# mathematiguy/pypardis

Hardware: AMD Instinct MI355X
Metric: points clustered/sec (whole node), 100M 3-D pts, 1/2/4/8 GPUs; % HBM roofline (higher is better)
Workload: dtype f32 coords, f64 predicate

## Files before the change

pypardis_amd/csrc/engine.hip:

```cpp
#include <cstring>
#include <rocprim/rocprim.hpp>
#ifndef PD_SORT_ROCPRIM
#define PD_SORT_ROCPRIM 0
#endif

#include <algorithm>
#include <type_traits>
#include <cmath>
#include <cstring>
#include <vector>

#include "compact.hpp"
#include "internal.hpp"
#include "pred.hpp"
#include "rsort.hpp"
#include "scan.hpp"
#include "stream.hpp"
#include "uf.hpp"

namespace pd {
namespace {

#ifndef PD_CHECK_BOUNDS
#define PD_CHECK_BOUNDS 0
// ... 1130 lines not shown
            R.lim_lo = -(int32_t)(c < 64 ? c : 64);
            const int64_t up = g.nc[0] - 1 - c;
            R.lim_hi = (int32_t)(up < 64 ? up : 64);
        } else {
            const float csf = (float)g.cs[j];
            const float shrink = 1.0f - 1.0f / 65536.0f, abs_s = csf * (1.0f / 1048576.0f);
            float dl = fmaxf(f * csf * shrink - abs_s, 0.0f);
            float dh = fmaxf((1.0f - f) * csf * shrink - abs_s, 0.0f);
            if constexpr (M == 0) {
                dl *= dl;
                dh *= dh;
            }
            R.tl[j] = c > 0 ? dl : INFINITY;
            R.th[j] = c < g.nc[j] - 1 ? dh : INFINITY;
        }
    }
    R.kc = g.base + lin;
    return R;
}

template <typename T, int D, int M, bool U>
__device__ __forceinline__ void row_range3(const Cells& C, const Count3Grid<T, D, M, U>& g,
                                           const RowGeo<D>& R, float e2, int q, uint32_t& s,
                                           uint32_t& e) {
    float d2 = 0.0f;
    int64_t koff = 0;
#pragma unroll
    for (int j = 1; j < D; ++j) {
        const int o = row_off<D>(q, j);
        d2 += o < 0 ? R.tl[j] : (o > 0 ? R.th[j] : 0.0f);
        koff += o < 0 ? -(int64_t)g.S[j] : (o > 0 ? (int64_t)g.S[j] : 0);
    }
    const bool ok = d2 <= e2;
    float w;
    if constexpr (M == 0)
        w = fmaxf(__builtin_amdgcn_sqrtf(fmaxf(e2 - d2, 0.0f)), 1.0842022e-19f);
    else
        w = fmaxf(e2 - d2, 0.0f);
    const float wc = w * g.wsc + g.wsl;
    int32_t dx0 = (int32_t)floorf(R.f0 - wc), dx1 = (int32_t)floorf(R.f0 + wc);
    dx0 = dx0 > R.lim_lo ? dx0 : R.lim_lo;
    dx1 = dx1 < R.lim_hi ? dx1 : R.lim_hi;
    const uint64_t rb = R.kc + (uint64_t)koff;
    const uint64_t k0 = ok ? rb + (uint64_t)(int64_t)dx0 : R.kc;
    const uint64_t k1 = ok ? rb + (uint64_t)(int64_t)(dx1 + 1) : R.kc;
    const uint4 w0 = dir_word(C, k0), w1 = dir_word(C, k1);
    const uint32_t i0 = dir_rank(w0, k0), i1 = dir_rank(w1, k1);
    s = C.cstart[i0];
    e = C.cstart[i1];
    e = e > s ? e : s;
}

#ifndef PD_COUNT_WPE
#define PD_COUNT_WPE 8
#endif
#ifndef PD_BORDER_WPE
#define PD_BORDER_WPE 8
#endif
constexpr int kCountWpe = PD_COUNT_WPE, kBorderWpe = PD_BORDER_WPE;
template <typename T, int D, int M, bool ST, int WPE = 1, bool REPLAY = false, bool WT = false>
__global__ __launch_bounds__(kBlock) __attribute__((amdgpu_waves_per_eu(WPE))) void count4_kernel(
    const T* __restrict__ Xs, uint32_t R, Cells C, double eps, double eps2, float lo, float hi,
    uint32_t ms, int full, uint32_t rot_min, uint8_t* __restrict__ core,
    uint32_t* __restrict__ mn_out, uint32_t* __restrict__ cnt_out,
    unsigned long long* __restrict__ stats, uint32_t rmod,
    const uint64_t* __restrict__ wrec = nullptr, uint64_t wthr = 0) {
    constexpr int NR = NRows<D>::v;
    constexpr int B = NR < 3 ? NR : 3, NB = NR / B;
    uint32_t r = rec_index();
    if (r >= R) return;
    if constexpr (REPLAY) r = r % rmod;
    (void)rmod;
    double a[D];
    load_rec<T, D>(Xs, r, a);
    const Pred<T, D, M> pr = make_pred<T, D, M>(Xs, r, a, eps, eps2, lo, hi);
    const uint32_t stop = full ? 0xFFFFFFFFu : ms;
    float e2 = M == 0 ? (float)eps2 : (float)eps;
    e2 = e2 * (1.0f + 1.0f / 65536.0f);
    uint32_t cnt = 0, mn = kNone, mn2 = kNone, n_cand = 0;
    uint64_t wsum = 0;
    const uint64_t wstop = full ? ~0ull : wthr;
    (void)wsum;
    (void)wstop;
    with_part(C.part_start, C.P, r, [&](int L, auto U) {
        Count3Grid<T, D, M, decltype(U)::value> g;
        g.load(C.parts + L);
        const RowGeo<D> geo = row_geo<T, D, M, decltype(U)::value>(g, a);
        for (int bt = 0; bt < NB; ++bt) {
            uint32_t s0, e0, s1 = 0, e1 = 0, s2 = 0, e2r = 0;
            row_range3<T, D, M, decltype(U)::value>(C, g, geo, e2, bt * B, s0, e0);
            if constexpr (B > 1) row_range3<T, D, M, decltype(U)::value>(C, g, geo, e2, bt * B + 1, s1, e1);
            if constexpr (B > 2) row_range3<T, D, M, decltype(U)::value>(C, g, geo, e2, bt * B + 2, s2, e2r);
            const uint32_t l0 = e0 - s0, l01 = l0 + (e1 - s1), tot = l01 + (e2r - s2);
            auto jpos = [&](uint32_t w) -> uint32_t {
                uint32_t j = s0 + w;
                if constexpr (B > 1) j = w >= l0 ? s1 + (w - l0) : j;
                if constexpr (B > 2) j = w >= l01 ? s2 + (w - l01) : j;
                return j;
            };
            uint32_t v0 = 0;
            if (bt == 0 && tot > rot_min) {
                const uint32_t vr = (r & ~(kRotAlign - 1u)) - s0;
                v0 = vr < l0 ? vr : 0u;
            }
            auto sweep = [&](auto ROT) -> bool {
                for (uint32_t v = 0; v < tot; v += 4) {
                    uint32_t j[4];
                    T b[4][D];
                    uint64_t wb[4];
                    (void)wb;
#pragma unroll
                    for (int u = 0; u < 4; ++u) {
                        uint32_t w = v + u;
                        if constexpr (decltype(ROT)::value) {
                            w += v0;
                            w = w >= tot ? w - tot : w;
                        }
                        j[u] = jpos(w);
                        load_raw<T, D>(Xs, v + u < tot ? j[u] : r, b[u]);
                        if constexpr (WT) wb[u] = wrec[v + u < tot ? j[u] : r];
                    }
#pragma unroll
                    for (int u = 0; u < 4; ++u) {
                        const bool h = (v + u < tot) && pr(b[u]);
                        cnt += h ? 1u : 0u;
                        if constexpr (WT) wsum += h ? wb[u] : 0ull;
                        const uint32_t x = h ? j[u] : kNone;
                        mn2 = min(mn2, max(mn, x));
                        mn = min(mn, x);
                    }
                    if constexpr (ST) n_cand += (tot - v < 4u ? tot - v : 4u);
                    if constexpr (WT) {
                        if (wsum >= wstop) return true;
                    } else {
                        if (cnt >= stop) return true;
                    }
                }
                return false;
            };
            const bool stopped = __any(v0 != 0) ? sweep(std::true_type{}) : sweep(std::false_type{});
            if (stopped) return;
        }
    });
    const bool is_core = WT ? wsum >= wthr : cnt >= ms;
    core[r] = (is_core ? 1 : 0) | (cnt >= 2 ? 2 : 0) | (cnt == 2 ? 4 : 0);
    reinterpret_cast<uint2*>(mn_out)[r] = make_uint2(mn, mn2);
    if constexpr (!WT)
        if (cnt_out) cnt_out[r] = full ? cnt : (cnt < ms ? cnt : ms);
    if constexpr (ST) atomicAdd(stats + 0, (unsigned long long)n_cand);
}

constexpr uint32_t kMixed = 0xFFFFFFFEu;

__device__ __forceinline__ uint32_t root_l1(const uint32_t* par, uint32_t x) {
    uint32_t p = ld_l1(par + x);
    while (p != x) {
        x = p;
        p = ld_l1(par + x);
    }
    return x;
}

__device__ __forceinline__ uint32_t lds_find(const uint32_t* lp, uint32_t x) {
    uint32_t p = lp[x];
    while (p != x) {
        x = p;
        p = lp[x];
    }
    return x;
}

__device__ __forceinline__ void lds_union(uint32_t* lp, uint32_t a, uint32_t b) {
    while (true) {
        a = lds_find(lp, a);
        b = lds_find(lp, b);
        if (a == b) return;
        if (a > b) {
            const uint32_t t = a;
            a = b;
            b = t;
        }
        if (atomicCAS(lp + b, b, a) == b) return;
    }
}

template <typename T, int D, int M, int W, bool ST>
__global__ __launch_bounds__(kBlock) void window_uf_kernel(const T* __restrict__ Xs, uint32_t R,
                                                           double eps, double eps2, float lo,
                                                           float hi, uint32_t* __restrict__ par,
                                                           unsigned long long* __restrict__ stats) {
    constexpr int E = 64 + W;
    static_assert(E <= 128, "two slots per lane");
    __shared__ T sx[kBlock / 64][E][D];
    __shared__ uint32_t sp[kBlock / 64][E];
    __shared__ uint32_t lp[kBlock / 64][E];
    const int lane = threadIdx.x & 63, w = threadIdx.x >> 6;
    const uint32_t b = xcd_block(blockIdx.x, gridDim.x) * kBlock + w * 64;
    for (int e = lane; e < E; e += 64) {
        const uint32_t j = b + e;
        T v[D];
        uint32_t p = kNone;
        if (j < R) {
            load_raw<T, D>(Xs, j, v);
            p = ld_l1(par + j);
            if (p != kNone && p != j) {
                const uint32_t root = root_l1(par, p);
                if (e < 64 && root != p) st_rlx(par + j, root);
                p = root;
            }
        } else {
#pragma unroll
            for (int k = 0; k < D; ++k) v[k] = T(0);
        }
#pragma unroll
        for (int k = 0; k < D; ++k) sx[w][e][k] = v[k];
        sp[w][e] = p;
        lp[w][e] = (uint32_t)e;
    }
    __syncthreads();
    const uint32_t r = b + lane;
    const uint32_t p0 = r < R ? sp[w][lane] : kNone;
    LinkStats st;
    if (p0 != kNone) {
        Pred<T, D, M> pr;
#pragma unroll
        for (int k = 0; k < D; ++k) {
            pr.ar[k] = sx[w][lane][k];
            pr.a[k] = (double)pr.ar[k];
        }
        pr.eps = eps;
        pr.eps2 = eps2;
        pr.lo = lo;
        pr.hi = hi;
#pragma unroll 4
        for (int k = 1; k <= W; ++k) {
            const uint32_t pj = sp[w][lane + k];
            if (pj == kNone || pj == p0 || r + k >= R) continue;
            T bj[D];
#pragma unroll
            for (int q = 0; q < D; ++q) bj[q] = sx[w][lane + k][q];
            if constexpr (ST) ++st.cand;
            if (pr(bj)) {
                if constexpr (ST) ++st.hit;
                lds_union(lp[w], (uint32_t)lane, (uint32_t)(lane + k));
            }
        }
    }
    __syncthreads();
    for (int e = lane; e < E; e += 64) {
        const uint32_t pe = sp[w][e];
        if (pe == kNone) continue;
        const uint32_t lr = lds_find(lp[w], (uint32_t)e);
        const uint32_t pl = sp[w][lr];
        if (pl == pe) continue;
        if (e > 0 && sp[w][e - 1] == pe && lds_find(lp[w], (uint32_t)(e - 1)) == lr) continue;
        if constexpr (ST) ++st.unions;
        uf_link_roots(par, uf_find_l1(par, pl), uf_find_l1(par, pe));
    }
    if constexpr (ST) {
        const uint32_t c = block_sum_u32(st.cand), h = block_sum_u32(st.hit),
                       u = block_sum_u32(st.unions);
        if (threadIdx.x == 0) {
            atomicAdd(stats + 1, (unsigned long long)c);
            atomicAdd(stats + 2, (unsigned long long)h);
            atomicAdd(stats + 6, (unsigned long long)u);
        }
    }
}

__device__ __forceinline__ uint32_t root_merge(uint32_t a, uint32_t b) {
    return a == kNone ? b : (b == kNone ? a : (a == b ? a : kMixed));
}

__device__ __forceinline__ uint32_t core_root(uint32_t* __restrict__ par, uint32_t r) {
    const uint32_t p0 = par[r];
    if (p0 == kNone) return kNone;
    uint32_t p = p0;
    while (true) {
        const uint32_t q = par[p];
        if (q == p) break;
        p = q;
    }
    if (p != p0) par[r] = p;
    return p;
}

__device__ __forceinline__ void word_merge(uint32_t* wroot, uint64_t w, uint32_t v) {
    if (v == kNone) return;
    uint32_t cur = ld_rlx(wroot + w);
    while (true) {
        const uint32_t want = root_merge(cur, v);
        if (want == cur) return;
        const uint32_t prev = atomicCAS(wroot + w, cur, want);
        if (prev == cur) return;
        cur = prev;
    }
}

constexpr uint32_t kMidCell = 16, kWordBig = 1024;

template <typename K, bool W32>
__global__ __launch_bounds__(kBlock) void cell_word_root_kernel(
    const uint32_t* __restrict__ cstart, const uint32_t* __restrict__ ncells,
    const K* __restrict__ ckeys, uint32_t* __restrict__ par, uint32_t* __restrict__ croot,
    uint32_t* __restrict__ wroot, uint32_t* __restrict__ mid, uint32_t* __restrict__ nmid,
    uint32_t* __restrict__ big, uint32_t* __restrict__ nbig, const uint4* __restrict__ pages) {
    const uint32_t c = blockIdx.x * kBlock + threadIdx.x;
    const int lane = threadIdx.x & 63;
    const uint32_t nc = *ncells;
    if (c - (uint32_t)lane >= nc) return;
    using WT = std::conditional_t<W32, uint32_t, uint64_t>;
    uint32_t v = kNone;
    WT word = (WT)~0ull;
    uint32_t sz = 0, s = 0;
    if (c < nc) {
        s = cstart[c];
        sz = cstart[c + 1] - s;
        word = (WT)word_slot(pages, (uint64_t)ckeys[c]);
    }
    wave_append(mid, nmid, sz > kMidCell && sz <= kWordBig, c);
    wave_append(big, nbig, sz > kWordBig, c);
    if (c < nc && sz <= kMidCell) {
        for (uint32_t b = s; b < s + sz; b += 4) {
            uint32_t p0[4], p1[4];
#pragma unroll
            for (int q = 0; q < 4; ++q) p0[q] = b + q < s + sz ? par[b + q] : kNone;
#pragma unroll
            for (int q = 0; q < 4; ++q) p1[q] = p0[q] != kNone ? par[p0[q]] : kNone;
#pragma unroll
            for (int q = 0; q < 4; ++q) {
                if (p0[q] == kNone) continue;
                uint32_t x = p0[q];
                if (p1[q] != x) {
                    x = p1[q];
                    while (true) {
                        const uint32_t y = par[x];
                        if (y == x) break;
                        x = y;
                    }
                    par[b + q] = x;
                }
                v = root_merge(v, x);
            }
        }
        croot[c] = v;
    }
#pragma unroll
    for (int o = 1; o < 64; o <<= 1) {
        const uint32_t nv = (uint32_t)__shfl_up((int)v, o, 64);
        const WT nw = shfl_up_w(word, o);
        if (lane >= o && nw == word) v = root_merge(v, nv);
    }
    const WT next = shfl_down_w(word, 1);
    if (c < nc && (lane == 63 || next != word)) word_merge(wroot, (uint64_t)word, v);
}

template <typename K>
__global__ __launch_bounds__(kBlock) void mid_cell_word_root_kernel(
    const uint32_t* __restrict__ cstart, const K* __restrict__ ckeys,
    const uint32_t* __restrict__ mid, const uint32_t* __restrict__ nmid,
    uint32_t* __restrict__ par, uint32_t* __restrict__ croot, uint32_t* __restrict__ wroot,
    const uint4* __restrict__ pages) {
    const uint32_t lane = threadIdx.x & 63;
    const uint32_t nm = *nmid;
    const uint32_t nw = gridDim.x * (kBlock / 64);
    for (uint32_t i = (blockIdx.x * kBlock + threadIdx.x) >> 6; i < nm; i += nw) {
        const uint32_t c = mid[i];
        const uint32_t s = cstart[c], e = cstart[c + 1];
        uint32_t v = kNone;
        for (uint32_t r = s + lane; r < e; r += 64) v = root_merge(v, core_root(par, r));
#pragma unroll
        for (int o = 32; o > 0; o >>= 1) v = root_merge(v, (uint32_t)__shfl_xor((int)v, o, 64));
        if (lane == 0) {
            croot[c] = v;
            word_merge(wroot, word_slot(pages, (uint64_t)ckeys[c]), v);
        }
    }
}

template <typename K>
__global__ __launch_bounds__(kBlock) void big_cell_word_root_kernel(
    const uint32_t* __restrict__ cstart, const K* __restrict__ ckeys,
    const uint32_t* __restrict__ big, const uint32_t* __restrict__ nbig,
    uint32_t* __restrict__ par, uint32_t* __restrict__ croot, uint32_t* __restrict__ wroot,
    const uint4* __restrict__ pages) {
    __shared__ uint32_t part[kBlock / 64];
    const uint32_t nb = *nbig;
    for (uint32_t i = blockIdx.x; i < nb; i += gridDim.x) {
        const uint32_t c = big[i];
        const uint32_t e = cstart[c + 1];
        uint32_t v = kNone;
        for (uint32_t r = cstart[c] + threadIdx.x; r < e; r += kBlock) v = root_merge(v, core_root(par, r));
#pragma unroll
        for (int o = 32; o > 0; o >>= 1) v = root_merge(v, (uint32_t)__shfl_xor((int)v, o, 64));
        if ((threadIdx.x & 63) == 0) part[threadIdx.x >> 6] = v;
        __syncthreads();
        if (threadIdx.x == 0) {
            uint32_t w = kNone;
#pragma unroll
            for (int k = 0; k < kBlock / 64; ++k) w = root_merge(w, part[k]);
            croot[c] = w;
            word_merge(wroot, word_slot(pages, (uint64_t)ckeys[c]), w);
        }
        __syncthreads();
// ... 793 lines not shown
    } else {
        PD_HIP(hipMemsetAsync(cstart, 0, sizeof(uint32_t), s));
        PD_HIP(hipMemsetAsync(dncells, 0, sizeof(uint32_t), s));
    }
    uint64_t cgrid0 = R;
#if PD_NC_SYNC
    if (R) {
        uint32_t* hnc = (uint32_t*)((char*)pinned(ctx, 16) + 8);
        PD_HIP(hipMemcpyAsync(hnc, dncells, sizeof(uint32_t), hipMemcpyDeviceToHost, s));
        uint32_t* hwb = hnc + 1;
        if (wbad) PD_HIP(hipMemcpyAsync(hwb, wbad, sizeof(uint32_t), hipMemcpyDeviceToHost, s));
        sync(s);
        cgrid0 = std::max<uint64_t>(1, std::min<uint64_t>(*hnc, R));
        if (wbad && *hwb)
            throw Error(-1, "sample_weight: " + std::to_string(*hwb) +
                                " value(s) not finite or outside [0, 2^31]");
        wbad = nullptr;
    }
#endif
    if (wbad) {
        uint32_t* hwb = (uint32_t*)pinned(ctx, sizeof(uint32_t));
        PD_HIP(hipMemcpyAsync(hwb, wbad, sizeof(uint32_t), hipMemcpyDeviceToHost, s));
        sync(s);
        if (*hwb)
            throw Error(-1, "sample_weight: " + std::to_string(*hwb) +
                                " value(s) not finite or outside [0, 2^31]");
    }
    auto prefix_words = [&](uint4* d, uint64_t nw, bool read_total) -> uint64_t {
        const unsigned wtiles = (unsigned)std::max<uint64_t>(1, (nw + 4 * kBlock - 1) / (4 * kBlock));
        uint32_t* wcnt = ctx.arena.get<uint32_t>("tile_cnt", (size_t)wtiles + 1);
        uint64_t* woff = ctx.arena.get<uint64_t>("tile_off", (size_t)wtiles + 1);
        hipLaunchKernelGGL(dir_tile_kernel, dim3(wtiles), dim3(kBlock), 0, s, d, nw, wcnt);
        const uint64_t tot = tile_offsets(ctx, wcnt, wtiles, woff, s, read_total);
        hipLaunchKernelGGL(dir_write_kernel, dim3(wtiles), dim3(kBlock), 0, s, d, nw, woff);
        return tot;
    };
    uint64_t W;
    uint4* dir;
    uint4* pages = nullptr;
    if (!a.dir_paged) {
        W = (Gtot >> 6) + 2;
        dir = ctx.arena.get<uint4>("dir", W);
        PD_HIP(hipMemsetAsync(dir, 0, sizeof(uint4) * W, s));
        if (R) {
            if (sizeof(K) == 4 || key_bits <= 37)
                hipLaunchKernelGGL((dir_bits_kernel<K, 0, true>), dim3(blocks(cgrid0)), dim3(kBlock), 0, s,
                                   ckeys, dncells, dir);
            else
                hipLaunchKernelGGL((dir_bits_kernel<K, 0, false>), dim3(blocks(cgrid0)), dim3(kBlock), 0,
                                   s, ckeys, dncells, dir);
        }
        prefix_words(dir, W, false);
    } else {
        const uint64_t NP = (Gtot >> 12) + 2;
        pages = ctx.arena.get<uint4>("dir_pages", NP);
        PD_HIP(hipMemsetAsync(pages, 0, sizeof(uint4) * NP, s));
        if (R) {
            if (sizeof(K) == 4 || key_bits <= 43)
                hipLaunchKernelGGL((dir_bits_kernel<K, 6, true>), dim3(blocks(cgrid0)), dim3(kBlock), 0, s,
                                   ckeys, dncells, pages);
            else
                hipLaunchKernelGGL((dir_bits_kernel<K, 6, false>), dim3(blocks(cgrid0)), dim3(kBlock), 0,
                                   s, ckeys, dncells, pages);
        }
        if (R && !PD_NC_SYNC)
            PD_HIP(hipMemcpyAsync((char*)pinned(ctx, 16) + 8, dncells, sizeof(uint32_t),
                                  hipMemcpyDeviceToHost, s));
        const uint64_t nw = prefix_words(pages, NP, true);
        W = nw + 1;
        dir = ctx.arena.get<uint4>("dir", W);
        if (R)
        {
            const uint32_t nch = *(const uint32_t*)((const char*)pinned(ctx, 16) + 8);
            const uint64_t wg = std::max<uint64_t>(1, std::min<uint64_t>(nch, R));
            if (sizeof(K) == 4 || key_bits <= 37)
                hipLaunchKernelGGL((word_write_kernel<K, true>), dim3(blocks(wg)), dim3(kBlock), 0, s,
                                   ckeys, dncells, pages, dir);
            else
                hipLaunchKernelGGL((word_write_kernel<K, false>), dim3(blocks(wg)), dim3(kBlock), 0, s,
                                   ckeys, dncells, pages, dir);
        }
        else
            PD_HIP(hipMemsetAsync(dir, 0, sizeof(uint4), s));
    }
    ctx.t.dir_words = (int64_t)W;
    PD_HIP(hipGetLastError());
    tm.mark();

    Cells C{parts, part_start, P, dir, cstart, pages};
    const double eps = a.eps, eps2 = a.eps * a.eps;
    float slo = -1.0f, shi = INFINITY;
    {
        const double thr = a.metric == 0 ? eps2 : eps;
        if (std::is_same<T, float>::value && thr > 1e-30 && thr < 1e30 && ctx.screen) {
            slo = std::nextafter((float)(thr * (1.0 - 1.0 / 262144.0)), 0.0f);
            shi = std::nextafter((float)(thr * (1.0 + 1.0 / 262144.0)), INFINITY);
        }
    }
    uint8_t* core = ctx.arena.get<uint8_t>("core", R);
    uint32_t* mn = ctx.arena.get<uint32_t>("minnbr", 2 * (size_t)R);
    uint32_t* cnt_rec = a.counts ? ctx.arena.get<uint32_t>("cnt_rec", R) : nullptr;
    unsigned long long* sst = nullptr;
    if (ctx.sweep_stats) {
        sst = ctx.arena.get<unsigned long long>("sweep_stats", 10);
        PD_HIP(hipMemsetAsync(sst, 0, sizeof(unsigned long long) * 10, s));
    }
    uint32_t* h_nc = nullptr;
    hipEvent_t ev_nc = nullptr;
    if (R && ctx.centre_window < 0) {
        h_nc = (uint32_t*)pinned(ctx, sizeof(uint32_t));
        PD_HIP(hipEventCreateWithFlags(&ev_nc, hipEventDisableTiming));
        PD_HIP(hipMemcpyAsync(h_nc, dncells, sizeof(uint32_t), hipMemcpyDeviceToHost, s));
        PD_HIP(hipEventRecord(ev_nc, s));
    }
    if (R) {
        const uint32_t rot = ctx.count_rotate ? (uint32_t)ctx.count_rotate : 0xFFFFFFFFu;
        if (wrec)
            launch_count_weighted<T, D, M>(s, Xs, R, C, eps, eps2, slo, shi, (uint32_t)a.min_samples,
                                           ctx.full_counts ? 1 : 0, rot, core, mn, wrec);
        else if (sst)
            launch_count<T, D, M, true>(s, Xs, R, C, eps, eps2, slo, shi, (uint32_t)a.min_samples,
                                        ctx.full_counts ? 1 : 0, rot, core, mn, cnt_rec, sst);
        else
            launch_count<T, D, M, false>(s, Xs, R, C, eps, eps2, slo, shi, (uint32_t)a.min_samples,
                                         ctx.full_counts ? 1 : 0, rot, core, mn, cnt_rec, sst);
        if (ctx.count_replay > 0 && !sst && !wrec)
            ctx.t.count_kernel = replay_count<T, D, M>(
                s, Xs, R, (uint32_t)ctx.count_replay, C, eps, eps2, slo, shi,
                (uint32_t)a.min_samples, ctx.full_counts ? 1 : 0, rot, core, mn, cnt_rec);
    }
    PD_HIP(hipGetLastError());
    tm.mark();

    uint32_t* par = ctx.arena.get<uint32_t>("parent", R);
    uint32_t* gmin = ctx.arena.get<uint32_t>("gmin", R);
    if (R) {
        uint32_t* wroot = ctx.arena.get<uint32_t>("word_root", W);
        const uint64_t NW = a.phase == 0 ? (n + 31) / 32 : 0;
        const uint64_t NWz = NW ? ((NW + 31) & ~uint64_t(31)) + kRootLists * kRootCntStride : 0;
        uint32_t* kbits = NW ? ctx.arena.get<uint32_t>("key_bits", NWz) : nullptr;
        hipLaunchKernelGGL(init_kernel, dim3(sub_blocks(std::max<uint64_t>(std::max<uint64_t>(R, W), NWz))),
                           dim3(kBlock), 0, s, R, core, mn, 1, par, gmin, wroot, (uint64_t)W, kbits, NWz);
        int cw = ctx.centre_window;
        uint64_t cgrid = R;
        if (cw < 0) {
            PD_HIP(hipEventSynchronize(ev_nc));
            (void)hipEventDestroy(ev_nc);
            const uint32_t nc = *h_nc ? *h_nc : 1u;
            cgrid = std::min<uint64_t>(nc, R);
            cw = 2 * (uint64_t)R <= 5ull * nc ? 2 : ((uint64_t)R <= 8ull * nc ? 8 : 16);
        }
        auto go = [&](auto Wc) {
            constexpr int Wv = decltype(Wc)::value;
            if (sst)
                hipLaunchKernelGGL((window_uf_kernel<T, D, M, Wv, true>), dim3(blocks(R)),
                                   dim3(kBlock), 0, s, Xs, R, eps, eps2, slo, shi, par, sst);
            else
                hipLaunchKernelGGL((window_uf_kernel<T, D, M, Wv, false>), dim3(blocks(R)),
                                   dim3(kBlock), 0, s, Xs, R, eps, eps2, slo, shi, par, sst);
        };
        if (cw <= 2)
            go(std::integral_constant<int, 2>{});
        else if (cw <= 4)
            go(std::integral_constant<int, 4>{});
        else if (cw <= 8)
            go(std::integral_constant<int, 8>{});
        else if (cw <= 16)
            go(std::integral_constant<int, 16>{});
        else if (cw <= 32)
            go(std::integral_constant<int, 32>{});
        else
            go(std::integral_constant<int, 64>{});
        uint32_t* croot = ctx.arena.get<uint32_t>("cell_root", R);
        {
            uint32_t* big = ctx.arena.get<uint32_t>("big_cells", R / (kWordBig + 1) + 1);
            uint32_t* mid = ctx.arena.get<uint32_t>("mid_cells", R / (kMidCell + 1) + 1);
            uint32_t* nbig = ctrs + 8;
            if ((uint64_t)W < 0xFFFFFFFFull)
                hipLaunchKernelGGL((cell_word_root_kernel<K, true>), dim3(blocks(cgrid)), dim3(kBlock), 0,
                                   s, cstart, dncells, ckeys, par, croot, wroot, mid, nbig + 1, big,
                                   nbig, pages);
            else
                hipLaunchKernelGGL((cell_word_root_kernel<K, false>), dim3(blocks(cgrid)), dim3(kBlock),
                                   0, s, cstart, dncells, ckeys, par, croot, wroot, mid, nbig + 1,
                                   big, nbig, pages);
            hipLaunchKernelGGL((mid_cell_word_root_kernel<K>), dim3(2048), dim3(kBlock), 0, s,
                               cstart, ckeys, mid, nbig + 1, par, croot, wroot, pages);
            hipLaunchKernelGGL((big_cell_word_root_kernel<K>), dim3(1024), dim3(kBlock), 0, s,
                               cstart, ckeys, big, nbig, par, croot, wroot, pages);
        }
        const uint32_t pcap = (uint32_t)std::min<uint64_t>(R, 64ull << 20);
        uint2* plist = ctx.arena.get<uint2>("pair_list", pcap);
        uint32_t* pcount = ctrs + 10;
        const unsigned vtiles = blocks(cgrid);
        uint8_t* vflag = ctx.arena.get<uint8_t>("verify_flags", R);
        uint32_t* vlist = ctx.arena.get<uint32_t>("verify_list", R);
        uint32_t* vcnt = ctx.arena.get<uint32_t>("tile_cnt", (size_t)vtiles + 1);
        uint64_t* voff = ctx.arena.get<uint64_t>("tile_off", (size_t)vtiles + 1);
        if (ctx.verify_fused) {
            hipLaunchKernelGGL((cell_verify_kernel<T, D, M, K>), dim3(vtiles), dim3(kBlock), 0, s,
                               Xs, keys, nullptr, 0u, croot, wroot, C, xsub_of(ctx), eps, eps2,
                               slo, shi, par, plist, pcap, pcount, sst, dncells);
        } else {
            hipLaunchKernelGGL((verify_screen_kernel<D, K>), dim3(vtiles), dim3(kBlock), 0, s, keys,
                               dncells, croot, wroot, C, xsub_of(ctx), vflag, vcnt);
            const uint32_t NV = (uint32_t)tile_offsets(ctx, vcnt, vtiles, voff, s, true);
            if (NV) {
                hipLaunchKernelGGL(flag_list_kernel, dim3(vtiles), dim3(kBlock), 0, s, vflag, dncells,
                                   voff, vlist);
                hipLaunchKernelGGL((cell_verify_kernel<T, D, M, K>), dim3(blocks(NV)), dim3(kBlock), 0,
                                   s, Xs, keys, vlist, NV, croot, wroot, C, xsub_of(ctx), eps, eps2,
                                   slo, shi, par, plist, pcap, pcount, sst, nullptr);
            }
        }
        hipLaunchKernelGGL((pair_kernel<T, D, M>), dim3(std::min(blocks(pcap), 4096u)), dim3(kBlock), 0, s, Xs, plist,
                           pcount, pcap, cstart, croot, eps, eps2, slo, shi, par);
    }
    PD_HIP(hipGetLastError());
    tm.mark();
    if (P > 1 && R) {
        const unsigned gb = std::min(blocks(R), 2048u);
        hipLaunchKernelGGL(rep_kernel, dim3(gb), dim3(kBlock), 0, s, dup_list, lcount, vals, par,
                           rep);
        hipLaunchKernelGGL(merge_kernel, dim3(gb), dim3(kBlock), 0, s, dup_list, lcount, vals, rep,
                           par);
    }
    tm.mark();
    if (R) {
        const unsigned rb = sub_blocks(R, kRootSub);
        const uint32_t seg = ((rb + kRootLists - 1) / kRootLists) * (uint32_t)(kRootSub * kBlock);
        const uint64_t NW = a.phase == 0 ? (n + 31) / 32 : 0;
        uint32_t* rlist = NW ? ctx.arena.get<uint32_t>("root_list", (size_t)seg * kRootLists) : nullptr;
        uint32_t* rcnt = NW ? ctx.arena.get<uint32_t>("key_bits", 1) + ((NW + 31) & ~uint64_t(31))
                            : nullptr;
        hipLaunchKernelGGL(roots_kernel, dim3(rb), dim3(kBlock), 0, s, R, vals, a.gid, par, gmin, rlist,
                           rcnt, seg, lcount + 1, ctx.sweep_stats ? 1 : 0);
        if (a.phase == 0) {
            uint32_t* kbits = ctx.arena.get<uint32_t>("key_bits", 1);
            uint32_t* kpre = ctx.arena.get<uint32_t>("key_pre", NW);
            const unsigned gb = kRootLists * 16;
            hipLaunchKernelGGL(root_mark_kernel, dim3(gb), dim3(kBlock), 0, s, rlist, rcnt, seg, gmin,
                               kbits);
            rocprim::transform_iterator<const uint32_t*, PopcOp, uint32_t> pc(kbits, PopcOp{});
            size_t tb = 0;
            PD_HIP(rocprim::exclusive_scan(nullptr, tb, pc, kpre, 0u, (size_t)NW,
                                           rocprim::plus<uint32_t>(), s));
            void* tmp = ctx.arena.get<char>("key_scan_tmp", tb);
            PD_HIP(rocprim::exclusive_scan(tmp, tb, pc, kpre, 0u, (size_t)NW,
                                           rocprim::plus<uint32_t>(), s));
            hipLaunchKernelGGL(root_rank_kernel, dim3(gb), dim3(kBlock), 0, s, rlist, rcnt, seg, kbits,
                               kpre, NW, gmin, lcount + 1);
        } else if (ctx.sweep_stats) {
            uint32_t* h = (uint32_t*)pinned(ctx, sizeof(uint32_t) * 4);
            PD_HIP(hipMemcpyAsync(h, lcount + 2, sizeof(uint32_t), hipMemcpyDeviceToHost, s));
            sync(s);
            ctx.t.core_records = h[0];
        }
    }
    ctx.st.n_roots = 0;
    PD_HIP(hipGetLastError());
    tm.mark();

    PhaseState& st = ctx.st;
    st.R = R;
    st.n = n;
    st.G = Gtot;
    st.P = P;
    st.d = D;
    st.dtype = std::is_same<T, float>::value ? 0 : 1;
    st.metric = M;
    st.min_samples = a.min_samples;
    st.key_bits = key_bits;
    st.eps = a.eps;
    st.slo = slo;
    st.shi = shi;
    st.Xs = Xs;
    st.parts = parts;
    st.part_start = part_start;
    st.dir = dir;
    st.pages = pages;
    st.cstart = cstart;
    st.vals = vals;
    st.core = core;
    st.par = par;
    st.gmin = gmin;
    st.cnt_rec = cnt_rec;
    st.mn = mn;
    st.n_exports = 0;
    if (a.phase == 1 && R && a.xr) {
        uint32_t* elist = nullptr;
        const uint32_t NE = select_records(ctx, "export_list", R, IsExport{core, vals, a.xr},
                                           &elist, s);
        st.exp_gid = ctx.arena.get<uint32_t>("exp_gid", NE + 1);
        st.exp_key = ctx.arena.get<uint32_t>("exp_key", NE + 1);
        if (NE)
            hipLaunchKernelGGL(export_kernel, dim3(blocks(NE)), dim3(kBlock), 0, s, NE, elist, vals,
                               par, gmin, a.gid, st.exp_gid, st.exp_key);
        PD_HIP(hipGetLastError());
        st.n_exports = NE;
    }
    a.n_exports = st.n_exports;
    st.valid = true;
}


template <typename T, int D, int M>
void run_b(Ctx& ctx, TrainArgs& a, EvTimer& tm) {
    hipStream_t s = a.stream;
    PhaseState& st = ctx.st;
    const uint64_t n = st.n;
    const uint32_t R = st.R;
    const T* Xs = (const T*)st.Xs;
// ... 433 lines not shown
```

Baseline: 4.193 billion.

## Process multiple 64-row groups per wave in window union-find kernel

Each wave in the window union-find kernel now covers K×64 rows (K picked at compile time from an LDS budget), so the W-row look-ahead halo is loaded once per K groups instead of once per 64 rows. The per-element serial root chase is replaced by a wave-wide loop that walks all of a lane's slots together, issuing their parent loads side by side. The launch grid shrinks by K to match. This raises LDS use per block and register pressure, which may lower occupancy.

```diff
diff --git a/pypardis_amd/csrc/engine.hip b/pypardis_amd/csrc/engine.hip
--- a/pypardis_amd/csrc/engine.hip
+++ b/pypardis_amd/csrc/engine.hip
@@ -1306,15 +1306,6 @@
 
 constexpr uint32_t kMixed = 0xFFFFFFFEu;
 
-__device__ __forceinline__ uint32_t root_l1(const uint32_t* par, uint32_t x) {
-    uint32_t p = ld_l1(par + x);
-    while (p != x) {
-        x = p;
-        p = ld_l1(par + x);
-    }
-    return x;
-}
-
 __device__ __forceinline__ uint32_t lds_find(const uint32_t* lp, uint32_t x) {
     uint32_t p = lp[x];
     while (p != x) {
@@ -1338,72 +1329,114 @@
     }
 }
 
+
+#ifndef PD_WINDOW_GROUPS
+#define PD_WINDOW_GROUPS 4
+#endif
+#ifndef PD_WINDOW_LDS
+#define PD_WINDOW_LDS 5851
+#endif
+static_assert(PD_WINDOW_LDS * (kBlock / 64) <= 65536, "a block's static LDS");
+
+constexpr int window_groups(int elem, int D, int W) {
+    int k = 1;
+    while (2 * k <= PD_WINDOW_GROUPS && (64 * 2 * k + W) * (elem * D + 8) <= PD_WINDOW_LDS) k *= 2;
+    return k;
+}
+
 template <typename T, int D, int M, int W, bool ST>
 __global__ __launch_bounds__(kBlock) void window_uf_kernel(const T* __restrict__ Xs, uint32_t R,
                                                            double eps, double eps2, float lo,
                                                            float hi, uint32_t* __restrict__ par,
                                                            unsigned long long* __restrict__ stats) {
-    constexpr int E = 64 + W;
-    static_assert(E <= 128, "two slots per lane");
+    constexpr int K = window_groups((int)sizeof(T), D, W);
+    constexpr int E = 64 * K + W;
+    constexpr int S = (E + 63) / 64;
+    static_assert(W >= 1 && W <= 64, "one look-ahead slot per lane");
     __shared__ T sx[kBlock / 64][E][D];
     __shared__ uint32_t sp[kBlock / 64][E];
     __shared__ uint32_t lp[kBlock / 64][E];
     const int lane = threadIdx.x & 63, w = threadIdx.x >> 6;
-    const uint32_t b = xcd_block(blockIdx.x, gridDim.x) * kBlock + w * 64;
-    for (int e = lane; e < E; e += 64) {
+    const uint32_t b = xcd_block(blockIdx.x, gridDim.x) * (uint32_t)(kBlock * K) + w * (64 * K);
+    T v[S][D];
+    uint32_t p[S], p0[S];
+#pragma unroll
+    for (int i = 0; i < S; ++i) {
+        const int e = lane + 64 * i;
         const uint32_t j = b + e;
-        T v[D];
-        uint32_t p = kNone;
-        if (j < R) {
-            load_raw<T, D>(Xs, j, v);
-            p = ld_l1(par + j);
-            if (p != kNone && p != j) {
-                const uint32_t root = root_l1(par, p);
-                if (e < 64 && root != p) st_rlx(par + j, root);
-                p = root;
+        p0[i] = kNone;
+#pragma unroll
+        for (int k = 0; k < D; ++k) v[i][k] = T(0);
+        if (e < E && j >= b && j < R) {
+            load_raw<T, D>(Xs, j, v[i]);
+            p0[i] = ld_l1(par + j);
+        }
+    }
+    uint32_t open = 0;
+#pragma unroll
+    for (int i = 0; i < S; ++i) {
+        p[i] = p0[i];
+        if (p0[i] != kNone && p0[i] != b + (uint32_t)(lane + 64 * i)) open |= 1u << i;
+    }
+    while (__any(open != 0)) {
+        uint32_t q[S];
+#pragma unroll
+        for (int i = 0; i < S; ++i)
+            if (open >> i & 1u) q[i] = ld_l1(par + p[i]);
+#pragma unroll
+        for (int i = 0; i < S; ++i)
+            if (open >> i & 1u) {
+                if (q[i] == p[i]) open &= ~(1u << i);
+                p[i] = q[i];
             }
-        } else {
-#pragma unroll
-            for (int k = 0; k < D; ++k) v[k] = T(0);
-        }
-#pragma unroll
-        for (int k = 0; k < D; ++k) sx[w][e][k] = v[k];
-        sp[w][e] = p;
-        lp[w][e] = (uint32_t)e;
+    }
+#pragma unroll
+    for (int i = 0; i < S; ++i) {
+        const int e = lane + 64 * i;
+        if (i < K && p[i] != p0[i]) st_rlx(par + b + e, p[i]);
+        if (e < E) {
+#pragma unroll
+            for (int k = 0; k < D; ++k) sx[w][e][k] = v[i][k];
+            sp[w][e] = p[i];
+            lp[w][e] = (uint32_t)e;
+        }
     }
     __syncthreads();
-    const uint32_t r = b + lane;
-    const uint32_t p0 = r < R ? sp[w][lane] : kNone;
     LinkStats st;
-    if (p0 != kNone) {
-        Pred<T, D, M> pr;
+    Pred<T, D, M> pr;
+    pr.eps = eps;
+    pr.eps2 = eps2;
+    pr.lo = lo;
+    pr.hi = hi;
+#pragma unroll
+    for (int i = 0; i < K; ++i) {
+        if (p[i] == kNone) continue;
+        const int e = lane + 64 * i;
 #pragma unroll
         for (int k = 0; k < D; ++k) {
-            pr.ar[k] = sx[w][lane][k];
-            pr.a[k] = (double)pr.ar[k];
-        }
-        pr.eps = eps;
-        pr.eps2 = eps2;
-        pr.lo = lo;
-        pr.hi = hi;
+            pr.ar[k] = v[i][k];
+            pr.a[k] = (double)v[i][k];
+        }
 #pragma unroll 4
         for (int k = 1; k <= W; ++k) {
-            const uint32_t pj = sp[w][lane + k];
-            if (pj == kNone || pj == p0 || r + k >= R) continue;
+            const uint32_t pj = sp[w][e + k];
+            if (pj == kNone || pj == p[i]) continue;
             T bj[D];
 #pragma unroll
-            for (int q = 0; q < D; ++q) bj[q] = sx[w][lane + k][q];
+            for (int q = 0; q < D; ++q) bj[q] = sx[w][e + k][q];
             if constexpr (ST) ++st.cand;
             if (pr(bj)) {
                 if constexpr (ST) ++st.hit;
-                lds_union(lp[w], (uint32_t)lane, (uint32_t)(lane + k));
+                lds_union(lp[w], (uint32_t)e, (uint32_t)(e + k));
             }
         }
     }
     __syncthreads();
-    for (int e = lane; e < E; e += 64) {
-        const uint32_t pe = sp[w][e];
-        if (pe == kNone) continue;
+#pragma unroll
+    for (int i = 0; i < S; ++i) {
+        const int e = lane + 64 * i;
+        if (e >= E || p[i] == kNone) continue;
+        const uint32_t pe = p[i];
         const uint32_t lr = lds_find(lp[w], (uint32_t)e);
         const uint32_t pl = sp[w][lr];
         if (pl == pe) continue;
@@ -2503,12 +2536,14 @@
         }
         auto go = [&](auto Wc) {
             constexpr int Wv = decltype(Wc)::value;
+            constexpr int Kw = window_groups((int)sizeof(T), D, Wv);
+            const unsigned wb = blocks(((uint64_t)R + Kw - 1) / Kw);
             if (sst)
-                hipLaunchKernelGGL((window_uf_kernel<T, D, M, Wv, true>), dim3(blocks(R)),
-                                   dim3(kBlock), 0, s, Xs, R, eps, eps2, slo, shi, par, sst);
+                hipLaunchKernelGGL((window_uf_kernel<T, D, M, Wv, true>), dim3(wb), dim3(kBlock), 0,
+                                   s, Xs, R, eps, eps2, slo, shi, par, sst);
             else
-                hipLaunchKernelGGL((window_uf_kernel<T, D, M, Wv, false>), dim3(blocks(R)),
-                                   dim3(kBlock), 0, s, Xs, R, eps, eps2, slo, shi, par, sst);
+                hipLaunchKernelGGL((window_uf_kernel<T, D, M, Wv, false>), dim3(wb), dim3(kBlock), 0,
+                                   s, Xs, R, eps, eps2, slo, shi, par, sst);
         };
         if (cw <= 2)
             go(std::integral_constant<int, 2>{});
```

After: 4.303 billion (median of 6 runs). +2.6%, better.
